# Jumpat/SegAnyGAussians

Hardware: AMD Instinct MI355X
Metric: train views/sec (fwd+bwd), 1080p, 1M Gaussians, 32-D features (higher is better)
Workload: dtype f32; 1 GPU; BASELINE cfg3: 1000000 Gaussians, 1920x1080, 32-D features, fwd+bwd, 1 view/GPU/step; parallelism=view-sharded x1

## Files before the change

### seganygaussians_amd/csrc/bin_full.h

```cpp
#pragma once

#include "blend_rec.h"
#include "common.h"
#include "cull.h"
#include "wave.h"

namespace mirast {

constexpr int BIN_MAX_WG = 256;
constexpr int BIN_THREADS = 1024;
constexpr int BIN_MAX_TILES = 22 * 1024 - 64;

__device__ __forceinline__ uint32_t slice_row(uint32_t b, uint32_t nwg)
{
    return (nwg & 7u) ? b : (b & 7u) * (nwg >> 3) + (b >> 3);
}

struct RectWork {
    uint32_t* prefix;
    uint32_t* rx;
    uint32_t* ry;
    uint32_t* wsum;
};

// ... 74 lines not shown
                getRect(rec.xy.x, rec.xy.y, (int)rec.pm, rmin, rmax, gx, gy);
                rmin.y = max(rmin.y, by0);
                rmax.y = min(rmax.y, by1);
                count = rmax.y > rmin.y ? (rmax.x - rmin.x) * (rmax.y - rmin.y) : 0u;
                s_xy[tid] = rec.xy;
                s_co[tid] = rec.co;
                s_rad[tid] = rec.pm;
                s_key[tid] = key;
            }
        }
        for_each_tile_balanced(rw, tid, rmin, rmax, count, [&](uint32_t owner, uint32_t tx, uint32_t ty) {
            const uint32_t qmask = NOCULL ? 15u : span_tile_mask(s_xy[owner], s_co[owner], (int)s_rad[owner], tx, ty, gx, gy);
            const uint32_t id = (uint32_t)(((it * 16 + (int)(owner >> 6)) * nwg + (int)blockIdx.x) * 64 + (int)(owner & 63u));
            const uint32_t slot = atomicAdd(&s_cnt[(ty - by0) * gx + tx], 1u);
            entries[slot] = make_uint2(s_key[owner], id | (qmask << ID_BITS));
        });
    }
}

__global__ void __launch_bounds__(BIN_THREADS) bin_count_kernel(int P, const BlendRec* __restrict__ index_rec,
                                                                const uint32_t* __restrict__ depth_key,
                                                                uint32_t* __restrict__ partial, uint32_t gx, uint32_t gy_all,
                                                                uint32_t by0, uint32_t by1, const int* __restrict__ r_slots,
                                                                int* __restrict__ host_r)
{
    extern __shared__ int s_grid[];
    const int tid = threadIdx.x, lane = tid & 63, wave = tid >> 6;
    if (host_r != nullptr && blockIdx.x == 0 && tid < R_SLOTS) host_r[tid * R_SLOT_STRIDE] = r_slots[tid * R_SLOT_STRIDE];
    const int stride = count_grid_stride(gx);
    const uint32_t gy = by1 - by0;
    const int cells = (int)(gy + 1) * stride;
    for (int c = tid; c < cells; c += BIN_THREADS) s_grid[c] = 0;
    __syncthreads();
    const int nwg = (int)gridDim.x;
    const int rounds = ((P + 63) / 64 + 16 * nwg - 1) / (16 * nwg);
    for (int it = 0; it < rounds; it++) {
        const int r = ((it * 16 + wave) * nwg + (int)blockIdx.x) * 64 + lane;
        if (r >= P) continue;
        if (depth_key[r] == 0xFFFFFFFFu) continue;
        const BlendRec rec = index_rec[r];
        uint2 rmin, rmax;
        getRect(rec.xy.x, rec.xy.y, (int)rec.pm, rmin, rmax, gx, gy_all);
        rmin.y = max(rmin.y, by0);
        rmax.y = min(rmax.y, by1);
        if (rmax.x <= rmin.x || rmax.y <= rmin.y) continue;
        rmin.y -= by0;
        rmax.y -= by0;
        atomicAdd(&s_grid[rmin.y * stride + rmin.x], 1);
        atomicAdd(&s_grid[rmin.y * stride + rmax.x], -1);
        atomicAdd(&s_grid[rmax.y * stride + rmin.x], -1);
        atomicAdd(&s_grid[rmax.y * stride + rmax.x], 1);
// ... 57 lines not shown
```

### seganygaussians_amd/csrc/bin_lean.h

```cpp
#pragma once

#include "blend_rec.h"
#include "common.h"
#include "cull.h"
#include "wave.h"

namespace mirast {

constexpr int BIN_LEAN_WG = 256;

__host__ __device__ inline bool band_geometry(uint32_t gx, uint32_t gy, uint32_t max_head_words, uint32_t& band_h, uint32_t& nbands)
{
    band_h = (gy + 15u) / 16u;
    if (band_h < 1u) band_h = 1u;
    while (band_h > 1u && (band_h + 1u) * (gx + 2u) > max_head_words) band_h--;
    nbands = (gy + band_h - 1u) / band_h;
    return nbands <= (uint32_t)MAX_BANDS && (band_h + 1u) * (gx + 2u) <= max_head_words;
}

__device__ __forceinline__ void band_plan(const int* __restrict__ r_slots, uint32_t nbands, uint32_t nwg, uint32_t* s_plan, int lane)
{
    uint32_t cnt = 0;
    if ((uint32_t)lane < nbands)
        for (int k = 0; k < R_SLOTS; k++) cnt += (uint32_t)r_slots[k * R_SLOT_STRIDE + R_SLOT_BANDS + lane];
    const uint32_t total = wave_sum(cnt);
    const uint32_t avail = nwg > nbands ? nwg - nbands : 0u;
    uint32_t n = (uint32_t)lane < nbands ? 1u + (total ? (uint32_t)(((uint64_t)cnt * avail) / total) : 0u) : 0u;
    if (nwg < nbands) n = (uint32_t)lane < nwg ? 1u : 0u;
    const uint32_t incl = wave_inclusive_scan(n, lane);
    if ((uint32_t)lane < nbands) s_plan[lane] = incl - n;
    if ((uint32_t)lane == nbands) s_plan[nbands] = incl;
}

constexpr int BW_WORDS = 64 * 18;
__host__ __device__ constexpr size_t span_lds_bytes(size_t head_words) { return (((head_words + 3) & ~(size_t)3) + 4 + 16 * BW_WORDS) * sizeof(uint32_t); }
constexpr uint32_t SPAN_MAX_HEAD_WORDS = 40 * 1024 - 16 * BW_WORDS - 64;

template <bool EMIT>
__global__ void __launch_bounds__(1024) bin_spans_kernel(int P, const BlendRec* __restrict__ index_rec,
                                                         const uint32_t* __restrict__ depth_key, const unsigned long long* __restrict__ band_bits,
                                                         uint32_t* __restrict__ partial, uint32_t* __restrict__ tile_total, const uint2* __restrict__ ranges,
                                                         uint2* __restrict__ entries, uint32_t gx, uint32_t gy_all,
                                                         uint32_t band_h, uint32_t nbands, const int* __restrict__ r_slots,
                                                         int* __restrict__ host_r)
{
    extern __shared__ uint32_t s_dyn[];
    __shared__ uint32_t s_plan[MAX_BANDS + 1];
    const int tid = threadIdx.x, lane = tid & 63, wave = tid >> 6;
    if (!EMIT && host_r != nullptr && blockIdx.x == 0 && tid < R_SLOTS) host_r[tid * R_SLOT_STRIDE] = r_slots[tid * R_SLOT_STRIDE];
    if (wave == 0) band_plan(r_slots, nbands, gridDim.x, s_plan, lane);
    __syncthreads();
    if (blockIdx.x >= s_plan[nbands]) return;
    uint32_t band = 0;
    while (band + 1u < nbands && s_plan[band + 1u] <= blockIdx.x) band++;
    const uint32_t nsub = s_plan[band + 1u] - s_plan[band], sub = blockIdx.x - s_plan[band];
    const uint32_t by0 = band * band_h, by1 = min(gy_all, by0 + band_h);
    const uint32_t band_bit = 1u << band;
    const uint32_t gy = by1 - by0;
    const int stride = count_grid_stride(gx);
    const int ntiles = (int)(gx * gy);
    const int tile0 = (int)(gx * by0);
    const int head = EMIT ? ((ntiles + 3) & ~3) : (((int)gy * stride + 3) & ~3);
    uint32_t* s_cnt = s_dyn;
    int* s_grid = reinterpret_cast<int*>(s_dyn);
    uint32_t* s_next = s_dyn + head;
    uint32_t* wb = s_dyn + head + 4 + wave * BW_WORDS;
    uint32_t* w_pre = wb;
    uint32_t* w_rect = wb + 64;
    uint32_t* w_key = wb + 128;
    uint32_t* w_own = wb + 192;
    float4* w_c0 = reinterpret_cast<float4*>(wb + 256);
    float4* w_c1 = reinterpret_cast<float4*>(wb + 512);
// ... 183 lines not shown
```

### seganygaussians_amd/csrc/common.h

```cpp
#pragma once

#include <hip/hip_runtime.h>
#include <stdint.h>

namespace mirast {

constexpr int R_SLOTS = 64;
constexpr int R_SLOT_STRIDE = 32;
constexpr int R_SLOT_BANDS = 4;
constexpr int MAX_BANDS = 24;
__host__ __device__ inline int count_grid_stride(uint32_t gx) { return (int)((gx + 1) | 1u); }


constexpr int TILE_X = 16;
constexpr int TILE_Y = 16;
constexpr int TILE_PIXELS = TILE_X * TILE_Y;
constexpr int BATCH = 256;
constexpr int WAVE = 64;

struct Mat3 {
    float m[3][3];
};

__device__ __forceinline__ Mat3 m3mul(const Mat3& A, const Mat3& B)
{
    Mat3 R;
#pragma unroll
    for (int c = 0; c < 3; c++)
#pragma unroll
        for (int r = 0; r < 3; r++)
            R.m[c][r] = A.m[0][r] * B.m[c][0] + A.m[1][r] * B.m[c][1] + A.m[2][r] * B.m[c][2];
    return R;
// ... 91 lines not shown
```

### seganygaussians_amd/csrc/geometry.h

```cpp
#pragma once

#include "blend_rec.h"
#include "common.h"
#include "wave.h"

namespace mirast {

__device__ constexpr float SH_C0 = 0.28209479177387814f;
__device__ constexpr float SH_C1 = 0.4886025119029199f;
__device__ constexpr float SH_C2[5] = {1.0925484305920792f, -1.0925484305920792f, 0.31539156525252005f,
                                       -1.0925484305920792f, 0.5462742152960396f};
__device__ constexpr float SH_C3[7] = {-0.5900435899266435f, 2.890611442640554f, -0.4570457994644658f,
                                       0.3731763325901154f, -0.4570457994644658f, 1.445305721320277f,
                                       -0.5900435899266435f};

__device__ __forceinline__ void computeCov3D(const float3 scale, float mod, const float4 rot, float* cov3D)
{
    Mat3 S = {{{1.0f, 0, 0}, {0, 1.0f, 0}, {0, 0, 1.0f}}};
    S.m[0][0] = mod * scale.x;
    S.m[1][1] = mod * scale.y;
    S.m[2][2] = mod * scale.z;
    float r = rot.x, x = rot.y, y = rot.z, z = rot.w;
    Mat3 R = {{{1.f - 2.f * (y * y + z * z), 2.f * (x * y - r * z), 2.f * (x * z + r * y)},
               {2.f * (x * y + r * z), 1.f - 2.f * (x * x + z * z), 2.f * (y * z - r * x)},
// ... 343 lines not shown
    for (int k = 0; k < 3; k++) {
        dL_dMt.m[0][k] *= s.x;
        dL_dMt.m[1][k] *= s.y;
        dL_dMt.m[2][k] *= s.z;
    }
    dL_drot.x = 2 * z * (dL_dMt.m[0][1] - dL_dMt.m[1][0]) + 2 * y * (dL_dMt.m[2][0] - dL_dMt.m[0][2]) + 2 * x * (dL_dMt.m[1][2] - dL_dMt.m[2][1]);
    dL_drot.y = 2 * y * (dL_dMt.m[1][0] + dL_dMt.m[0][1]) + 2 * z * (dL_dMt.m[2][0] + dL_dMt.m[0][2]) + 2 * r * (dL_dMt.m[1][2] - dL_dMt.m[2][1]) - 4 * x * (dL_dMt.m[2][2] + dL_dMt.m[1][1]);
    dL_drot.z = 2 * x * (dL_dMt.m[1][0] + dL_dMt.m[0][1]) + 2 * r * (dL_dMt.m[2][0] - dL_dMt.m[0][2]) + 2 * z * (dL_dMt.m[1][2] + dL_dMt.m[2][1]) - 4 * y * (dL_dMt.m[2][2] + dL_dMt.m[0][0]);
    dL_drot.w = 2 * r * (dL_dMt.m[0][1] - dL_dMt.m[1][0]) + 2 * x * (dL_dMt.m[2][0] + dL_dMt.m[0][2]) + 2 * y * (dL_dMt.m[1][2] + dL_dMt.m[2][1]) - 4 * z * (dL_dMt.m[1][1] + dL_dMt.m[0][0]);
}

__global__ void __launch_bounds__(256) geometry_bwd_kernel(
    int P, int D, int M, const float* __restrict__ means, const int* __restrict__ radii, const float* __restrict__ shs,
    const uint8_t* __restrict__ clamped, const float* __restrict__ scales, const float* __restrict__ rotations,
    const float* __restrict__ cov3Ds, ViewParams vp, const float* __restrict__ gpack ,
    float* __restrict__ dL_dmean2D, float* __restrict__ dL_dconics, float* __restrict__ dL_dopacity,
    float* __restrict__ dL_dmask, float* __restrict__ dL_dmeans, const float* __restrict__ dL_dcolor,
    float* __restrict__ dL_dcov, float* __restrict__ dL_dsh, float* __restrict__ dL_dscale, float* __restrict__ dL_drot)
{
    const int idx = blockIdx.x * blockDim.x + threadIdx.x;
    if (idx >= P) return;
    if (!(radii[idx] > 0)) {
        dL_dmean2D[3 * idx + 0] = dL_dmean2D[3 * idx + 1] = dL_dmean2D[3 * idx + 2] = 0.f;
        reinterpret_cast<float4*>(dL_dconics)[idx] = make_float4(0.f, 0.f, 0.f, 0.f);
        dL_dopacity[idx] = 0.f;
        if (dL_dmask) dL_dmask[idx] = 0.f;
#pragma unroll
        for (int i = 0; i < 6; i++) dL_dcov[(size_t)idx * 6 + i] = 0.f;
        dL_dmeans[3 * idx + 0] = dL_dmeans[3 * idx + 1] = dL_dmeans[3 * idx + 2] = 0.f;
        dL_dscale[3 * idx + 0] = dL_dscale[3 * idx + 1] = dL_dscale[3 * idx + 2] = 0.f;
        reinterpret_cast<float4*>(dL_drot)[idx] = make_float4(0.f, 0.f, 0.f, 0.f);
        return;
    }

    const float4 g0 = reinterpret_cast<const float4*>(gpack)[2 * idx];
    const float4 g1 = reinterpret_cast<const float4*>(gpack)[2 * idx + 1];
    dL_dmean2D[3 * idx + 0] = g0.x;
    dL_dmean2D[3 * idx + 1] = g0.y;
    dL_dmean2D[3 * idx + 2] = 0.f;
    reinterpret_cast<float4*>(dL_dconics)[idx] = make_float4(g0.z, g0.w, 0.f, g1.x);
    dL_dopacity[idx] = g1.y;
    if (dL_dmask) dL_dmask[idx] = g1.z;

    const float3 mean = make_float3(means[3 * idx], means[3 * idx + 1], means[3 * idx + 2]);
    const float3 dL_dconic = make_float3(g0.z, g0.w, g1.x);
    float cov3D[6];
#pragma unroll
    for (int i = 0; i < 6; i++) cov3D[i] = cov3Ds[(size_t)idx * 6 + i];
    Cov2DCtx c;
    cov2d_common(mean, vp, cov3D, c);
    const float h_x = vp.focal_x, h_y = vp.focal_y;
    const float limx = 1.3f * vp.tan_fovx;
    const float limy = 1.3f * vp.tan_fovy;
    const float x_grad_mul = c.txtz < -limx || c.txtz > limx ? 0 : 1;
    const float y_grad_mul = c.tytz < -limy || c.tytz > limy ? 0 : 1;
    const Mat3& T = c.T;
    const Mat3& Vrk = c.Vrk;
    const Mat3& Wm = c.W;
    const float3 t = c.t;
    const float a = c.cov.m[0][0];
    const float b = c.cov.m[0][1];
    const float cc = c.cov.m[1][1];
    const float denom = a * cc - b * b;
    float dL_da = 0, dL_db = 0, dL_dc = 0;
    const float denom2inv = 1.0f / ((denom * denom) + 0.0000001f);
    float dcov[6];
    if (denom2inv != 0) {
        dL_da = denom2inv * (-cc * cc * dL_dconic.x + 2 * b * cc * dL_dconic.y + (denom - a * cc) * dL_dconic.z);
        dL_dc = denom2inv * (-a * a * dL_dconic.z + 2 * a * b * dL_dconic.y + (denom - a * cc) * dL_dconic.x);
        dL_db = denom2inv * 2 * (b * cc * dL_dconic.x - (denom + 2 * b * b) * dL_dconic.y + a * b * dL_dconic.z);
        dcov[0] = (T.m[0][0] * T.m[0][0] * dL_da + T.m[0][0] * T.m[1][0] * dL_db + T.m[1][0] * T.m[1][0] * dL_dc);
        dcov[3] = (T.m[0][1] * T.m[0][1] * dL_da + T.m[0][1] * T.m[1][1] * dL_db + T.m[1][1] * T.m[1][1] * dL_dc);
        dcov[5] = (T.m[0][2] * T.m[0][2] * dL_da + T.m[0][2] * T.m[1][2] * dL_db + T.m[1][2] * T.m[1][2] * dL_dc);
        dcov[1] = 2 * T.m[0][0] * T.m[0][1] * dL_da + (T.m[0][0] * T.m[1][1] + T.m[0][1] * T.m[1][0]) * dL_db + 2 * T.m[1][0] * T.m[1][1] * dL_dc;
        dcov[2] = 2 * T.m[0][0] * T.m[0][2] * dL_da + (T.m[0][0] * T.m[1][2] + T.m[0][2] * T.m[1][0]) * dL_db + 2 * T.m[1][0] * T.m[1][2] * dL_dc;
        dcov[4] = 2 * T.m[0][2] * T.m[0][1] * dL_da + (T.m[0][1] * T.m[1][2] + T.m[0][2] * T.m[1][1]) * dL_db + 2 * T.m[1][1] * T.m[1][2] * dL_dc;
    } else {
#pragma unroll
        for (int i = 0; i < 6; i++) dcov[i] = 0;
    }
#pragma unroll
    for (int i = 0; i < 6; i++) dL_dcov[(size_t)idx * 6 + i] = dcov[i];

    const float dL_dT00 = 2 * (T.m[0][0] * Vrk.m[0][0] + T.m[0][1] * Vrk.m[0][1] + T.m[0][2] * Vrk.m[0][2]) * dL_da +
                          (T.m[1][0] * Vrk.m[0][0] + T.m[1][1] * Vrk.m[0][1] + T.m[1][2] * Vrk.m[0][2]) * dL_db;
    const float dL_dT01 = 2 * (T.m[0][0] * Vrk.m[1][0] + T.m[0][1] * Vrk.m[1][1] + T.m[0][2] * Vrk.m[1][2]) * dL_da +
                          (T.m[1][0] * Vrk.m[1][0] + T.m[1][1] * Vrk.m[1][1] + T.m[1][2] * Vrk.m[1][2]) * dL_db;
    const float dL_dT02 = 2 * (T.m[0][0] * Vrk.m[2][0] + T.m[0][1] * Vrk.m[2][1] + T.m[0][2] * Vrk.m[2][2]) * dL_da +
                          (T.m[1][0] * Vrk.m[2][0] + T.m[1][1] * Vrk.m[2][1] + T.m[1][2] * Vrk.m[2][2]) * dL_db;
    const float dL_dT10 = 2 * (T.m[1][0] * Vrk.m[0][0] + T.m[1][1] * Vrk.m[0][1] + T.m[1][2] * Vrk.m[0][2]) * dL_dc +
                          (T.m[0][0] * Vrk.m[0][0] + T.m[0][1] * Vrk.m[0][1] + T.m[0][2] * Vrk.m[0][2]) * dL_db;
    const float dL_dT11 = 2 * (T.m[1][0] * Vrk.m[1][0] + T.m[1][1] * Vrk.m[1][1] + T.m[1][2] * Vrk.m[1][2]) * dL_dc +
                          (T.m[0][0] * Vrk.m[1][0] + T.m[0][1] * Vrk.m[1][1] + T.m[0][2] * Vrk.m[1][2]) * dL_db;
    const float dL_dT12 = 2 * (T.m[1][0] * Vrk.m[2][0] + T.m[1][1] * Vrk.m[2][1] + T.m[1][2] * Vrk.m[2][2]) * dL_dc +
                          (T.m[0][0] * Vrk.m[2][0] + T.m[0][1] * Vrk.m[2][1] + T.m[0][2] * Vrk.m[2][2]) * dL_db;
    const float dL_dJ00 = Wm.m[0][0] * dL_dT00 + Wm.m[0][1] * dL_dT01 + Wm.m[0][2] * dL_dT02;
    const float dL_dJ02 = Wm.m[2][0] * dL_dT00 + Wm.m[2][1] * dL_dT01 + Wm.m[2][2] * dL_dT02;
    const float dL_dJ11 = Wm.m[1][0] * dL_dT10 + Wm.m[1][1] * dL_dT11 + Wm.m[1][2] * dL_dT12;
    const float dL_dJ12 = Wm.m[2][0] * dL_dT10 + Wm.m[2][1] * dL_dT11 + Wm.m[2][2] * dL_dT12;
    const float tz = 1.f / t.z;
    const float tz2 = tz * tz;
    const float tz3 = tz2 * tz;
    const float dL_dtx = x_grad_mul * -h_x * tz2 * dL_dJ02;
    const float dL_dty = y_grad_mul * -h_y * tz2 * dL_dJ12;
    const float dL_dtz = -h_x * tz2 * dL_dJ00 - h_y * tz2 * dL_dJ11 + (2 * h_x * t.x) * tz3 * dL_dJ02 + (2 * h_y * t.y) * tz3 * dL_dJ12;
// ... 43 lines not shown
```

### seganygaussians_amd/csrc/mi_rast.hip

```cpp
#include "host.h"

#include <algorithm>
#include <atomic>
#include <cstdio>
#include <cstdlib>
#include <cstring>
#include <mutex>
#include <type_traits>
#include <utility>
#include <vector>

#include "bin_full.h"
#include "bin_lean.h"
#include "tile_ranges.h"
#include "tile_sort.h"
#include "blend_bwd.h"
#include "blend_bwd_wave.h"
#include "blend_bwd_feat.h"
#include "blend_fwd.h"
#include "blend_fwd_wave.h"
#ifdef MI_RAST_PROFILING
#include "blend_fwd_x3.h"
#endif
#include "common.h"
#include "fingerprint.h"
#include "geometry.h"
// ... 1 lines not shown
#include "xcd_runs.h"
#include "xcd_stamp.h"

using namespace mirast;

namespace {

#define STAGE_CHECK(c, name)                                                                           \
    do {                                                                                               \
        hipError_t _e = hipGetLastError();                                                             \
        if (_e == hipSuccess && (c).debug) _e = hipStreamSynchronize((c).stream);                      \
        if (_e != hipSuccess)                                                                          \
            return fail(MI_RAST_ERR_HIP, std::string("[HIP ERROR] in stage ") + name + ": " + hipGetErrorString(_e)); \
    } while (0)

constexpr int MAX_DEVICES = 64;
struct HostSync {
    int* pinned = nullptr;
    int* pinned_dev = nullptr;
    uint64_t* fp = nullptr;
    uint64_t* fp_dev = nullptr;
    hipEvent_t ev = nullptr;
    hipEvent_t ev2 = nullptr;
    bool ok = false;
    const int* words() const { return pinned + R_SLOTS * R_SLOT_STRIDE; }
    int* words_dev() const { return pinned_dev + R_SLOTS * R_SLOT_STRIDE; }
    bool init()
    {
        if (ok) return true;
        if (hipHostMalloc((void**)&pinned, (R_SLOTS * R_SLOT_STRIDE + 16) * sizeof(int), hipHostMallocMapped) != hipSuccess) return false;
        if (hipHostGetDevicePointer((void**)&pinned_dev, pinned, 0) != hipSuccess) return false;
        if (hipHostMalloc((void**)&fp, (size_t)MI_FP_MAX * FP_BLOCKS * sizeof(uint64_t), hipHostMallocMapped) != hipSuccess) return false;
        if (hipHostGetDevicePointer((void**)&fp_dev, fp, 0) != hipSuccess) return false;
        if (hipEventCreateWithFlags(&ev, hipEventDisableTiming) != hipSuccess) return false;
        if (hipEventCreateWithFlags(&ev2, hipEventDisableTiming) != hipSuccess) return false;
        ok = true;
        return true;
    }
    ~HostSync()
    {
        if (ev) (void)hipEventDestroy(ev);
        if (ev2) (void)hipEventDestroy(ev2);
        if (pinned) (void)hipHostFree(pinned);
        if (fp) (void)hipHostFree(fp);
    }
};
thread_local HostSync g_host_sync_tl[MAX_DEVICES];
thread_local int g_last_longest_run[MAX_DEVICES];

int current_device()
{
    int dev = 0;
    if (hipGetDevice(&dev) != hipSuccess || dev < 0 || dev >= MAX_DEVICES) return -1;
    return dev;
// ... 289 lines not shown
    const int max_lds = (int)((BIN_MAX_TILES + 11 * 1024 + 16) * sizeof(uint32_t));
    HIP_TRY(hipFuncSetAttribute((const void*)bin_ranks_kernel<false>, hipFuncAttributeMaxDynamicSharedMemorySize, max_lds));
    HIP_TRY(hipFuncSetAttribute((const void*)bin_ranks_kernel<true>, hipFuncAttributeMaxDynamicSharedMemorySize, max_lds));
    HIP_TRY(hipFuncSetAttribute((const void*)bin_count_kernel, hipFuncAttributeMaxDynamicSharedMemorySize, max_lds));
    HIP_TRY(hipFuncSetAttribute((const void*)bin_spans_kernel<false>, hipFuncAttributeMaxDynamicSharedMemorySize, 160 * 1024 - 256));
    HIP_TRY(hipFuncSetAttribute((const void*)bin_spans_kernel<true>, hipFuncAttributeMaxDynamicSharedMemorySize, 160 * 1024 - 256));
    HIP_TRY(hipFuncSetAttribute((const void*)tile_ranges_kernel, hipFuncAttributeMaxDynamicSharedMemorySize,
                                (BIN_MAX_TILES_TOTAL + 1) * (int)sizeof(uint32_t)));
    g_attr_set[dev].store(true, std::memory_order_release);
    return MI_RAST_OK;
}

int count_and_scan_stage(const Call& c, const BinPlan& bp, const HostSync& hs)
{
    const int P = c.P, ntiles = (int)c.ntiles();
    {
        StageTimer t(c.stream, MI_STAGE_TILE_SCAN);
        if (bp.full) {
            const size_t cnt_lds = (size_t)(bp.band_rows + 1) * count_grid_stride(c.vp.grid_x) * sizeof(int);
            for (uint32_t b = 0; b < bp.nbands; b++) {
                const uint32_t by0 = b * bp.band_rows, by1 = std::min(c.vp.grid_y, by0 + bp.band_rows);
                hipLaunchKernelGGL(bin_count_kernel, dim3(bp.nwg), dim3(BIN_THREADS), cnt_lds, c.stream, P, c.geom.index_rec, c.geom.depth_key,
                                   c.img.tile_count, c.vp.grid_x, c.vp.grid_y, by0, by1, (const int*)c.img.num_rendered,
                                   b == 0 ? hs.pinned_dev : (int*)nullptr);
            }
        } else {
            hipLaunchKernelGGL(bin_spans_kernel<false>, dim3(bp.nwg), dim3(1024),
                               span_lds_bytes((size_t)bp.lean_band_h * count_grid_stride(c.vp.grid_x)), c.stream, P, c.geom.index_rec,
                               c.geom.depth_key, c.geom.band_bits, c.img.tile_count, c.img.tile_cursor, (const uint2*)nullptr, (uint2*)nullptr,
                               c.vp.grid_x, c.vp.grid_y, bp.lean_band_h, bp.lean_nbands, (const int*)c.img.num_rendered, hs.pinned_dev);
        }
        HIP_TRY(hipEventRecord(hs.ev, c.stream));
        if (bp.full)
            hipLaunchKernelGGL(scan_partials_kernel, dim3((ntiles + 63) / 64), dim3(1024), 0, c.stream, ntiles, bp.nwg,
                               c.img.tile_count, c.img.tile_cursor);
        const uint32_t run_cap = !(c.flags & MI_RAST_EQUAL_RUNS) ? (uint32_t)RUN_MODEL_CAP : 0u;
        hipLaunchKernelGGL(tile_ranges_kernel, dim3(1), dim3(1024),
                           ((size_t)std::min(ntiles, BIN_MAX_TILES_TOTAL) + 1) * sizeof(uint32_t), c.stream, ntiles, c.img.tile_cursor,
                           c.img.ranges, c.img.words(), (const int*)c.img.num_rendered, hs.words_dev(), c.img.tile_consumed, c.img.tile_nsurv,
                           c.img.run_bounds, run_cap, (uint32_t)RUN_MODEL_FIX);
    }
    STAGE_CHECK(c, "tile scan");
    return MI_RAST_OK;
}

int emit_stage(const Call& c, const BinPlan& bp, int R)
{
    const int P = c.P, ntiles = (int)c.ntiles();
    const bool verify = !bp.full && (c.flags & MI_RAST_VERIFY_LISTS) != 0;
    if (verify) HIP_TRY(hipMemsetAsync(c.bin.entries, 0, (size_t)R * sizeof(uint2), c.stream));
    {
        StageTimer t(c.stream, MI_STAGE_EMIT);
        if (bp.full) {
            const size_t band_tiles = (size_t)bp.band_rows * c.vp.grid_x;
            const size_t emit_lds = ((size_t)((band_tiles + 3) & ~(size_t)3) + 11 * 1024 + 16) * sizeof(uint32_t);
            for (uint32_t b = 0; b < bp.nbands; b++) {
                const uint32_t by0 = b * bp.band_rows, by1 = std::min(c.vp.grid_y, by0 + bp.band_rows);
                with_bool(bp.nocull, [&](auto nocull) {
                    hipLaunchKernelGGL(bin_ranks_kernel<decltype(nocull)::value>, dim3(bp.nwg), dim3(BIN_THREADS), emit_lds, c.stream, P, c.geom.index_rec,
                                       c.geom.depth_key, c.img.tile_count, c.img.ranges, c.bin.entries, c.vp.grid_x, c.vp.grid_y, by0, by1);
                });
            }
        } else {
            hipLaunchKernelGGL(bin_spans_kernel<true>, dim3(bp.nwg), dim3(1024), span_lds_bytes((size_t)bp.lean_band_h * c.vp.grid_x), c.stream,
                               P, c.geom.index_rec, c.geom.depth_key, c.geom.band_bits, c.img.tile_count, c.img.tile_cursor, c.img.ranges, c.bin.entries,
                               c.vp.grid_x, c.vp.grid_y, bp.lean_band_h, bp.lean_nbands, (const int*)c.img.num_rendered, (int*)nullptr);
        }
    }
    STAGE_CHECK(c, "emit entries");
    if (verify) {
        uint32_t* ctr = reinterpret_cast<uint32_t*>(c.img.words() + NR_VERIFY);
        HIP_TRY(hipMemsetAsync(ctr, 0, sizeof(uint32_t), c.stream));
        hipLaunchKernelGGL(verify_entries_kernel, dim3(ntiles), dim3(256), 0, c.stream, (uint32_t)ntiles, c.img.ranges, c.bin.entries, ctr);
        uint32_t unwritten = 0;
        HIP_TRY(hipMemcpyAsync(&unwritten, ctr, sizeof(uint32_t), hipMemcpyDeviceToHost, c.stream));
        HIP_TRY(hipStreamSynchronize(c.stream));
        if (unwritten)
            return fail(MI_RAST_ERR_HIP, "internal error: " + std::to_string(unwritten) + " list slots were counted but not emitted "
                                         "(count / emit passes of bin_spans_kernel disagree)");
    }
    return MI_RAST_OK;
}

int take_longest_run(Call& c, const HostSync& hs, int dev)
{
    HIP_TRY(hipEventSynchronize(hs.ev2));
    c.longest_run = longest_of(hs.words() + NR_RUN_BOUNDS, c.ntiles());
    g_last_longest_run[dev] = (int)c.longest_run;
    return MI_RAST_OK;
}

template <int CLASS>
void launch_tile_sort_wave(const Call& c)
{
    hipLaunchKernelGGL(tile_sort_wave_kernel<CLASS>, dim3((c.ntiles() + 3) / 4), dim3(256), 0, c.stream, c.ntiles(), c.img.ranges,
                       (const uint2*)c.bin.entries, c.bin.blend_list);
}
template <int LO, int CAP, bool FB, int NT>
void launch_tile_sort(const Call& c)
{
    hipLaunchKernelGGL((tile_sort_kernel<LO, CAP, FB, NT>), dim3(c.ntiles()), dim3(NT), 0, c.stream, c.ntiles(), c.img.ranges, c.bin.entries,
                       c.bin.scratch, (const int*)(c.img.words() + NR_KEY_BITS), c.bin.blend_list);
// ... 12 lines not shown
        if (max_tile_count > 2048) launch_tile_sort_wave<2>(c);
        if (max_tile_count > TILE_SORT_WAVE_MAX) launch_tile_sort<TILE_SORT_WAVE_MAX, 6144, false, 1024>(c);
        if (max_tile_count > 6144) launch_tile_sort<6144, 8192, true, 1024>(c);
    }
    STAGE_CHECK(c, "tile sort");
    return MI_RAST_OK;
}

int geometry_and_binning(Call& c, const FrontArgs& a, int* num_rendered)
{
    const int dev = current_device();
    if (dev < 0) return fail(MI_RAST_ERR_HIP, "hipGetDevice failed (or device ordinal >= 64)");
    HostSync& hs = g_host_sync_tl[dev];
    BinPlan bp;
    if (int rc = plan_binning(c, bp)) return rc;
    size_t goff[MI_GEOM_NFIELDS], ioff[MI_IMG_NFIELDS], boff[MI_BIN_NFIELDS];
    char* geom_base = a.geometry_buffer(mi_rast_geometry_layout(c.P, goff), a.geometry_user);
    if (!geom_base) return fail(MI_RAST_ERR_ALLOC, "geometry buffer callback returned NULL");
    c.geom = geom_from(geom_base, c.P);
    char* img_base = a.image_buffer(mi_rast_image_layout(c.vp.W, c.vp.H, ioff), a.image_user);
    if (!img_base) return fail(MI_RAST_ERR_ALLOC, "image buffer callback returned NULL");
    c.img = img_from(img_base, c.vp.W, c.vp.H);

    if (int rc = preprocess_stage(c, a, bp)) return rc;
    if (int rc = opt_in_to_large_lds(dev)) return rc;
    if (!hs.init()) return fail(MI_RAST_ERR_HIP, "cannot allocate pinned host buffer / event");
    if (int rc = count_and_scan_stage(c, bp, hs)) return rc;
    HIP_TRY(hipEventRecord(hs.ev2, c.stream));
    HIP_TRY(hipEventSynchronize(hs.ev));
    long long Rsum = 0;
    for (int k = 0; k < R_SLOTS; k++) Rsum += hs.pinned[k * R_SLOT_STRIDE];
    if (Rsum > 0x7fffffffll) return fail(MI_RAST_ERR_INVALID, "more than 2^31 tile overlaps");
    const int R = (int)Rsum;
    *num_rendered = R;

    char* bin_base = a.binning_buffer(mi_rast_binning_layout(R, boff), a.binning_user);
    if (!bin_base) return fail(MI_RAST_ERR_ALLOC, "binning buffer callback returned NULL");
    c.bin = bin_from(bin_base, R);
    if (R == 0) return take_longest_run(c, hs, dev);
    if (int rc = emit_stage(c, bp, R)) return rc;
    return sort_stage(c, bp, hs, dev, R);
}

struct FwdArgs { int channels; const float *features, *mask, *bg; float *out_color, *out_mask, *out_depth; };
struct BwdArgs { int channels; const float *bg, *colors, *dL_dpix, *dL_dout_mask; float* dL_dcolor; };

template <int C, int EXTRA>
void launch_blend_fwd(const Call& c, const FwdArgs& a, ChannelBlock b)
{
    constexpr bool MAY_BE_PARTIAL = C == 16 && EXTRA == 0;
    with_bools(MAY_BE_PARTIAL && b.real < C, c.xexp(), [&](auto partial, auto xexp) {
        if constexpr (MAY_BE_PARTIAL || !decltype(partial)::value)
            hipLaunchKernelGGL((blend_fwd_kernel<C, EXTRA, decltype(xexp)::value, decltype(partial)::value>), dim3(c.vp.grid_x, c.vp.grid_y), dim3(256), 0,
                               c.stream, c.img.ranges, c.bin.blend_list, c.geom.index_rec, c.vp.W, c.vp.H, a.features + b.c0, a.mask, c.geom.depths,
// ... 522 lines not shown
```

### seganygaussians_amd/rasterizer.py

```python
from __future__ import annotations

import contextlib
import math
import os
import ctypes as C
import threading
from typing import NamedTuple

import torch
import torch.nn as nn

from . import _lib
from ._ffi import check, contig, dev_ptr, stream_ptr
from .geometry_cache import GeometryCache, disable_geometry_cache, enable_geometry_cache, geometry_cache


def cpu_deep_copy_tuple(input_tuple):
    copied_tensors = [item.cpu().clone() if isinstance(item, torch.Tensor) else item for item in input_tuple]
    return tuple(copied_tensors)


class GaussianRasterizationSettings(NamedTuple):
    image_height: int
    image_width: int
# ... 181 lines not shown
    if background is None or background.numel() < channels:
        raise RuntimeError(f"bg must hold one value per channel: {0 if background is None else background.numel()} given, "
                           f"{channels} channels rendered")
    if colors is not None and colors.numel() != 0 and P != 0 and (colors.ndimension() != 2 or colors.size(0) != P
                                                                  or colors.size(1) != channels):
        raise RuntimeError(f"colors_precomp must have dimensions (num_points, {channels}); got {tuple(colors.shape)}")


def set_features_ready_event(event) -> None:
    _opts.features_ready = event


def _flags_of(geomBuffer, flags):
    if flags is not None:
        return flags
    notes = getattr(geomBuffer, "mi_notes", None)
    return 0 if notes is None else notes.flags


def rasterize_gaussians_backward_native(channels, with_mask_depth, background, means3D, radii, colors, scales,
                                        rotations, scale_modifier, cov3D_precomp, viewmatrix, projmatrix, tan_fovx,
                                        tan_fovy, dL_dout_color, dL_dout_mask, sh, degree, campos, geomBuffer, R,
                                        binningBuffer, imageBuffer, debug, flags=None, prezeroed=None, pack_zeroed=None,
                                        features_only=False):
    L = _lib.load()
    P = means3D.size(0)
    H, W = dL_dout_color.size(1), dL_dout_color.size(2)
    M = sh.size(1) if sh.numel() != 0 else 0
    dev = means3D.device
    _check_widths(channels, background, colors, P)
    if dL_dout_color.ndimension() != 3 or dL_dout_color.size(0) != channels:
        raise RuntimeError(f"dL_dout_color must have dimensions ({channels}, H, W); got {tuple(dL_dout_color.shape)}")
    if features_only and (with_mask_depth or colors.numel() == 0):
        raise RuntimeError("features_only backward needs precomputed colours and the plain (not DEPTH) rasterizer")
    full = not features_only
    o = dict(device=dev, dtype=torch.float32)
    g = {}
    if full:
        shapes = [("dL_dmeans3D", (P, 3)), ("dL_dmeans2D", (P, 3)), ("dL_dconic", (P, 2, 2)), ("dL_dopacity", (P, 1)),
                  ("dL_dcov3D", (P, 6)), ("dL_dscales", (P, 3)), ("dL_drotations", (P, 4))]
        if with_mask_depth:
            shapes.append(("dL_dmask", (P, 1)))
        counts = [math.prod(shp) for _, shp in shapes]
        starts = [0]
        for n in counts:
            starts.append(starts[-1] + (n + 3) // 4 * 4)
        flat = torch.empty(starts[-1], **o)
        if debug:
            flat.fill_(float("nan"))
        for (name, shp), n, off in zip(shapes, counts, starts):
            g[name] = flat[off:off + n].view(shp)
    if pack_zeroed is None:
        pack_zeroed = prezeroed is not None
    if prezeroed is not None and (tuple(prezeroed.shape) != (P, channels) or prezeroed.device != dev or (debug and full)):
        prezeroed = None
    g["dL_dcolors"] = prezeroed if prezeroed is not None else torch.zeros((P, channels), **o)
    if full:
        g["dL_dsh"] = torch.zeros((P, M, 3), **o)
    if P != 0:
        def only_full(x):
            return x if full else None

        def grad(name, present=True):
            return g[name].data_ptr() if (present and name in g) else None

        t = [contig(x) for x in (background, means3D, only_full(sh), colors, only_full(scales), only_full(rotations),
                                  only_full(cov3D_precomp), viewmatrix, projmatrix, campos, dL_dout_color,
                                  dL_dout_mask if with_mask_depth else None, radii)]
        bg_c, m3_c, sh_c, col_c, sc_c, rot_c, cov_c, vm_c, pm_c, cp_c, dpix_c, dmask_c, radii_c = t
        with torch.cuda.device(dev):
            rc = L.mi_rast_backward(
                P, int(degree), int(M) if full else 0, int(channels), int(R), dev_ptr(bg_c, "bg", dev), W, H,
                dev_ptr(m3_c, "means3D", dev), dev_ptr(sh_c, "sh", dev), dev_ptr(col_c, "colors_precomp", dev),
                dev_ptr(sc_c, "scales", dev), float(scale_modifier), dev_ptr(rot_c, "rotations", dev),
                dev_ptr(cov_c, "cov3D_precomp", dev), dev_ptr(vm_c, "viewmatrix", dev),
                dev_ptr(pm_c, "projmatrix", dev), dev_ptr(cp_c, "campos", dev), float(tan_fovx), float(tan_fovy),
                dev_ptr(radii_c, "radii", dev, torch.int32), geomBuffer.data_ptr(), binningBuffer.data_ptr(),
                imageBuffer.data_ptr(), dev_ptr(dpix_c, "dL_dout_color", dev), dev_ptr(dmask_c, "dL_dout_mask", dev),
                grad("dL_dmeans2D"), grad("dL_dconic"), grad("dL_dopacity"), grad("dL_dcolors"), grad("dL_dmask"),
                grad("dL_dmeans3D"), grad("dL_dcov3D"), grad("dL_dsh", M > 0), grad("dL_dscales"), grad("dL_drotations"),
                int(bool(debug)) if full else 0,
                int(_flags_of(geomBuffer, flags)) | (0 if full else _lib.MI_RAST_BWD_FEATURES_ONLY)
                | (_lib.MI_RAST_PREZERO_BWD if pack_zeroed else 0), stream_ptr(dev))
        check(rc)
    if features_only:
        return None, g["dL_dcolors"], None, None, None, None, None, None
    if with_mask_depth:
        return (g["dL_dmeans2D"], g["dL_dcolors"], g["dL_dopacity"], g["dL_dmask"], g["dL_dmeans3D"], g["dL_dcov3D"], g["dL_dsh"],
                g["dL_dscales"], g["dL_drotations"])
    return (g["dL_dmeans2D"], g["dL_dcolors"], g["dL_dopacity"], g["dL_dmeans3D"], g["dL_dcov3D"], g["dL_dsh"], g["dL_dscales"],
            g["dL_drotations"])


def mark_visible_native(means3D, viewmatrix, projmatrix):
    L = _lib.load()
    P = means3D.size(0)
    dev = means3D.device
    present = torch.zeros(P, dtype=torch.bool, device=dev)
    if P != 0:
        m3_c, vm_c, pm_c = contig(means3D), contig(viewmatrix), contig(projmatrix)
        with torch.cuda.device(dev):
            rc = L.mi_rast_mark_visible(P, dev_ptr(m3_c, "means3D", dev), dev_ptr(vm_c, "viewmatrix", dev),
                                        dev_ptr(pm_c, "projmatrix", dev), present.data_ptr(), stream_ptr(dev))
        check(rc)
    return present


def rasterize_mask_gaussians_native(means3D, opacity, mask, scales, rotations, scale_modifier, cov3D_precomp,
                                    viewmatrix, projmatrix, tan_fovx, tan_fovy, image_height, image_width,
                                    prefiltered, debug):
    _opts.features_ready = None
    if means3D.ndimension() != 2 or means3D.size(1) != 3:
        raise RuntimeError("means3D must have dimensions (num_points, 3)")
# ... 109 lines not shown
                                  binningBuffer, imgBuffer)
            ctx.mark_non_differentiable(radii)
            ctx.set_materialize_grads(False)
            ctx.out_shape = tuple(color.shape)
            return color, radii

        @staticmethod
        def backward(ctx, grad_out_color, _):
            num_rendered = ctx.num_rendered
            rs = ctx.raster_settings
            if grad_out_color is None:
                grad_out_color = torch.zeros(ctx.out_shape, dtype=torch.float32, device=ctx.saved_tensors[1].device)
            (colors_precomp, means3D, scales, rotations, cov3Ds_precomp, radii, sh, geomBuffer, binningBuffer,
             imgBuffer) = ctx.saved_tensors
            args = (rs.bg, means3D, radii, colors_precomp, scales, rotations, rs.scale_modifier, cov3Ds_precomp,
                    rs.viewmatrix, rs.projmatrix, rs.tanfovx, rs.tanfovy, grad_out_color, sh, rs.sh_degree, rs.campos,
                    geomBuffer, num_rendered, binningBuffer, imgBuffer, rs.debug)
            prezeroed, pack_zeroed = ctx.mi_notes.claim()
            feat_only = _features_only_applies(channels, colors_precomp, ctx.needs_input_grad, rs.debug)
            (grad_means2D, grad_colors_precomp, grad_opacities, grad_means3D, grad_cov3Ds_precomp, grad_sh,
             grad_scales, grad_rotations) = _snapshot_call(
                rs.debug, args, lambda *a: rasterize_gaussians_backward_native(
                    channels, False, *a[:13], None, *a[13:], flags=ctx.mi_notes.flags, prezeroed=prezeroed,
                    pack_zeroed=pack_zeroed, features_only=feat_only), *_SNAPSHOT_BW)
            return (grad_means3D, grad_means2D, grad_sh, grad_colors_precomp, grad_opacities, grad_scales,
                    grad_rotations, grad_cov3Ds_precomp, None)

    def rasterize_gaussians(means3D, means2D, sh, colors_precomp, opacities, scales, rotations, cov3Ds_precomp,
                            raster_settings):
        _opts.grad_mode = torch.is_grad_enabled()
        try:
            return _RasterizeGaussians.apply(means3D, means2D, sh, colors_precomp, opacities, scales, rotations,
                                             cov3Ds_precomp, raster_settings)
        finally:
            _opts.grad_mode = True

    class GaussianRasterizer(_RasterizerModule):
        def forward(self, means3D, means2D, opacities, shs=None, colors_precomp=None, scales=None, rotations=None,
                    cov3D_precomp=None):
            _one_of_colors(shs, colors_precomp)
            _one_of_cov(scales, rotations, cov3D_precomp)
            shs, colors_precomp, scales, rotations, cov3D_precomp = _or_empty(shs, colors_precomp, scales, rotations, cov3D_precomp)
            return rasterize_gaussians(means3D, means2D, shs, colors_precomp, opacities, scales, rotations,
                                       cov3D_precomp, self.raster_settings)

    return _RasterizeGaussians, rasterize_gaussians, GaussianRasterizer

# ... 18 lines not shown
            ctx.save_for_backward(colors_precomp, means3D, scales, rotations, cov3Ds_precomp, radii, sh, geomBuffer,
                                  binningBuffer, imgBuffer)
            ctx.mark_non_differentiable(radii)
            ctx.set_materialize_grads(False)
            ctx.out_shapes = (tuple(color.shape), tuple(out_mask.shape))
            return color, out_mask, depth, radii

        @staticmethod
        def backward(ctx, grad_out_color, grad_out_mask, grad_out_depth, _):
            num_rendered = ctx.num_rendered
            rs = ctx.raster_settings
            dev_ = ctx.saved_tensors[1].device
            if grad_out_color is None:
                grad_out_color = torch.zeros(ctx.out_shapes[0], dtype=torch.float32, device=dev_)
            if grad_out_mask is None:
                grad_out_mask = torch.zeros(ctx.out_shapes[1], dtype=torch.float32, device=dev_)
            (colors_precomp, means3D, scales, rotations, cov3Ds_precomp, radii, sh, geomBuffer, binningBuffer,
             imgBuffer) = ctx.saved_tensors
            args = (rs.bg, means3D, radii, colors_precomp, scales, rotations, rs.scale_modifier, cov3Ds_precomp,
                    rs.viewmatrix, rs.projmatrix, rs.tanfovx, rs.tanfovy, grad_out_color, grad_out_mask, sh,
                    rs.sh_degree, rs.campos, geomBuffer, num_rendered, binningBuffer, imgBuffer, rs.debug)
            (grad_means2D, grad_colors_precomp, grad_opacities, grad_mask, grad_means3D, grad_cov3Ds_precomp, grad_sh,
             grad_scales, grad_rotations) = _snapshot_call(
                rs.debug, args, lambda *a: rasterize_gaussians_backward_native(channels, True, *a, flags=ctx.mi_notes.flags),
                *_SNAPSHOT_BW)
            grad_mask = grad_mask.view(ctx.mask_shape)
            return (grad_means3D, grad_means2D, grad_sh, grad_colors_precomp, grad_opacities, grad_mask, grad_scales,
                    grad_rotations, grad_cov3Ds_precomp, None)

    class _RasterizeMaskGaussians(torch.autograd.Function):
        @staticmethod
        def forward(ctx, means3D, means2D, opacities, mask, scales, rotations, cov3Ds_precomp, raster_settings):
            rs = raster_settings
            num_rendered, out_mask, radii, geomBuffer, binningBuffer, imgBuffer = rasterize_mask_gaussians_native(
                means3D, opacities, mask, scales, rotations, rs.scale_modifier, cov3Ds_precomp, rs.viewmatrix,
                rs.projmatrix, rs.tanfovx, rs.tanfovy, rs.image_height, rs.image_width, rs.prefiltered, rs.debug)
            ctx.raster_settings = rs
            ctx.num_rendered = num_rendered
            ctx.mask_shape = mask.shape
            ctx.mi_notes = _take_notes(geomBuffer)
            ctx.save_for_backward(means3D, means2D, opacities, scales, rotations, cov3Ds_precomp, radii, geomBuffer,
                                  binningBuffer, imgBuffer)
            ctx.mark_non_differentiable(radii)
            ctx.set_materialize_grads(False)
            ctx.out_shape = tuple(out_mask.shape)
            return out_mask, radii

# ... 86 lines not shown
```

Before: 915.8 views/s.

## Poll generation-tagged pinned slots for num_rendered and skip unused conic/cov3D gradients

The count kernels now publish each per-slot rendered count to mapped host memory as a 64-bit word tagged with a generation number. The host spins briefly on those words instead of waiting on an event recorded after the count pass, falling back to the later event if the values do not arrive within the spin window. This is meant to shorten the forward-pass stall before the host learns the list size. Separately, the backward pass no longer allocates or writes the dL_dconic buffer, and skips dL_dcov3D when no precomputed covariances are supplied, which cuts memory traffic and allocation. The spin adds host CPU busy-waiting and relies on system-scope relaxed stores becoming visible in order.

```diff
diff --git a/seganygaussians_amd/csrc/bin_full.h b/seganygaussians_amd/csrc/bin_full.h
--- a/seganygaussians_amd/csrc/bin_full.h
+++ b/seganygaussians_amd/csrc/bin_full.h
@@ -120,11 +120,11 @@
                                                                 const uint32_t* __restrict__ depth_key,
                                                                 uint32_t* __restrict__ partial, uint32_t gx, uint32_t gy_all,
                                                                 uint32_t by0, uint32_t by1, const int* __restrict__ r_slots,
-                                                                int* __restrict__ host_r)
+                                                                int* __restrict__ host_r, uint32_t host_gen)
 {
     extern __shared__ int s_grid[];
     const int tid = threadIdx.x, lane = tid & 63, wave = tid >> 6;
-    if (host_r != nullptr && blockIdx.x == 0 && tid < R_SLOTS) host_r[tid * R_SLOT_STRIDE] = r_slots[tid * R_SLOT_STRIDE];
+    if (host_r != nullptr && blockIdx.x == 0 && tid < R_SLOTS) publish_r_slot(host_r, tid, r_slots[tid * R_SLOT_STRIDE], host_gen);
     const int stride = count_grid_stride(gx);
     const uint32_t gy = by1 - by0;
     const int cells = (int)(gy + 1) * stride;
diff --git a/seganygaussians_amd/csrc/bin_lean.h b/seganygaussians_amd/csrc/bin_lean.h
--- a/seganygaussians_amd/csrc/bin_lean.h
+++ b/seganygaussians_amd/csrc/bin_lean.h
@@ -42,12 +42,12 @@
                                                          uint32_t* __restrict__ partial, uint32_t* __restrict__ tile_total, const uint2* __restrict__ ranges,
                                                          uint2* __restrict__ entries, uint32_t gx, uint32_t gy_all,
                                                          uint32_t band_h, uint32_t nbands, const int* __restrict__ r_slots,
-                                                         int* __restrict__ host_r)
+                                                         int* __restrict__ host_r, uint32_t host_gen)
 {
     extern __shared__ uint32_t s_dyn[];
     __shared__ uint32_t s_plan[MAX_BANDS + 1];
     const int tid = threadIdx.x, lane = tid & 63, wave = tid >> 6;
-    if (!EMIT && host_r != nullptr && blockIdx.x == 0 && tid < R_SLOTS) host_r[tid * R_SLOT_STRIDE] = r_slots[tid * R_SLOT_STRIDE];
+    if (!EMIT && host_r != nullptr && blockIdx.x == 0 && tid < R_SLOTS) publish_r_slot(host_r, tid, r_slots[tid * R_SLOT_STRIDE], host_gen);
     if (wave == 0) band_plan(r_slots, nbands, gridDim.x, s_plan, lane);
     __syncthreads();
     if (blockIdx.x >= s_plan[nbands]) return;
diff --git a/seganygaussians_amd/csrc/common.h b/seganygaussians_amd/csrc/common.h
--- a/seganygaussians_amd/csrc/common.h
+++ b/seganygaussians_amd/csrc/common.h
@@ -8,6 +8,11 @@
 constexpr int R_SLOTS = 64;
 constexpr int R_SLOT_STRIDE = 32;
 constexpr int R_SLOT_BANDS = 4;
+__device__ __forceinline__ void publish_r_slot(int* host_r, int k, int partial_sum, uint32_t generation)
+{
+    const unsigned long long w = (unsigned long long)(uint32_t)partial_sum | ((unsigned long long)generation << 32);
+    __hip_atomic_store(reinterpret_cast<unsigned long long*>(host_r + k * R_SLOT_STRIDE), w, __ATOMIC_RELAXED, __HIP_MEMORY_SCOPE_SYSTEM);
+}
 constexpr int MAX_BANDS = 24;
 __host__ __device__ inline int count_grid_stride(uint32_t gx) { return (int)((gx + 1) | 1u); }
 
diff --git a/seganygaussians_amd/csrc/geometry.h b/seganygaussians_amd/csrc/geometry.h
--- a/seganygaussians_amd/csrc/geometry.h
+++ b/seganygaussians_amd/csrc/geometry.h
@@ -389,11 +389,13 @@
     if (idx >= P) return;
     if (!(radii[idx] > 0)) {
         dL_dmean2D[3 * idx + 0] = dL_dmean2D[3 * idx + 1] = dL_dmean2D[3 * idx + 2] = 0.f;
-        reinterpret_cast<float4*>(dL_dconics)[idx] = make_float4(0.f, 0.f, 0.f, 0.f);
+        if (dL_dconics) reinterpret_cast<float4*>(dL_dconics)[idx] = make_float4(0.f, 0.f, 0.f, 0.f);
         dL_dopacity[idx] = 0.f;
         if (dL_dmask) dL_dmask[idx] = 0.f;
-#pragma unroll
-        for (int i = 0; i < 6; i++) dL_dcov[(size_t)idx * 6 + i] = 0.f;
+        if (dL_dcov) {
+#pragma unroll
+            for (int i = 0; i < 6; i++) dL_dcov[(size_t)idx * 6 + i] = 0.f;
+        }
         dL_dmeans[3 * idx + 0] = dL_dmeans[3 * idx + 1] = dL_dmeans[3 * idx + 2] = 0.f;
         dL_dscale[3 * idx + 0] = dL_dscale[3 * idx + 1] = dL_dscale[3 * idx + 2] = 0.f;
         reinterpret_cast<float4*>(dL_drot)[idx] = make_float4(0.f, 0.f, 0.f, 0.f);
@@ -405,7 +407,7 @@
     dL_dmean2D[3 * idx + 0] = g0.x;
     dL_dmean2D[3 * idx + 1] = g0.y;
     dL_dmean2D[3 * idx + 2] = 0.f;
-    reinterpret_cast<float4*>(dL_dconics)[idx] = make_float4(g0.z, g0.w, 0.f, g1.x);
+    if (dL_dconics) reinterpret_cast<float4*>(dL_dconics)[idx] = make_float4(g0.z, g0.w, 0.f, g1.x);
     dL_dopacity[idx] = g1.y;
     if (dL_dmask) dL_dmask[idx] = g1.z;
 
@@ -446,8 +448,10 @@
 #pragma unroll
         for (int i = 0; i < 6; i++) dcov[i] = 0;
     }
-#pragma unroll
-    for (int i = 0; i < 6; i++) dL_dcov[(size_t)idx * 6 + i] = dcov[i];
+    if (dL_dcov) {
+#pragma unroll
+        for (int i = 0; i < 6; i++) dL_dcov[(size_t)idx * 6 + i] = dcov[i];
+    }
 
     const float dL_dT00 = 2 * (T.m[0][0] * Vrk.m[0][0] + T.m[0][1] * Vrk.m[0][1] + T.m[0][2] * Vrk.m[0][2]) * dL_da +
                           (T.m[1][0] * Vrk.m[0][0] + T.m[1][1] * Vrk.m[0][1] + T.m[1][2] * Vrk.m[0][2]) * dL_db;
diff --git a/seganygaussians_amd/csrc/mi_rast.hip b/seganygaussians_amd/csrc/mi_rast.hip
--- a/seganygaussians_amd/csrc/mi_rast.hip
+++ b/seganygaussians_amd/csrc/mi_rast.hip
@@ -2,6 +2,7 @@
 
 #include <algorithm>
 #include <atomic>
+#include <chrono>
 #include <cstdio>
 #include <cstdlib>
 #include <cstring>
@@ -49,7 +50,9 @@
     uint64_t* fp_dev = nullptr;
     hipEvent_t ev = nullptr;
     hipEvent_t ev2 = nullptr;
+    uint32_t generation = 0;
     bool ok = false;
+    uint32_t next_generation() { return ++generation ? generation : ++generation; }
     const int* words() const { return pinned + R_SLOTS * R_SLOT_STRIDE; }
     int* words_dev() const { return pinned_dev + R_SLOTS * R_SLOT_STRIDE; }
     bool init()
@@ -57,6 +60,7 @@
         if (ok) return true;
         if (hipHostMalloc((void**)&pinned, (R_SLOTS * R_SLOT_STRIDE + 16) * sizeof(int), hipHostMallocMapped) != hipSuccess) return false;
         if (hipHostGetDevicePointer((void**)&pinned_dev, pinned, 0) != hipSuccess) return false;
+        memset(pinned, 0, (R_SLOTS * R_SLOT_STRIDE + 16) * sizeof(int));
         if (hipHostMalloc((void**)&fp, (size_t)MI_FP_MAX * FP_BLOCKS * sizeof(uint64_t), hipHostMallocMapped) != hipSuccess) return false;
         if (hipHostGetDevicePointer((void**)&fp_dev, fp, 0) != hipSuccess) return false;
         if (hipEventCreateWithFlags(&ev, hipEventDisableTiming) != hipSuccess) return false;
@@ -392,15 +396,15 @@
                 const uint32_t by0 = b * bp.band_rows, by1 = std::min(c.vp.grid_y, by0 + bp.band_rows);
                 hipLaunchKernelGGL(bin_count_kernel, dim3(bp.nwg), dim3(BIN_THREADS), cnt_lds, c.stream, P, c.geom.index_rec, c.geom.depth_key,
                                    c.img.tile_count, c.vp.grid_x, c.vp.grid_y, by0, by1, (const int*)c.img.num_rendered,
-                                   b == 0 ? hs.pinned_dev : (int*)nullptr);
+                                   b == 0 ? hs.pinned_dev : (int*)nullptr, hs.generation);
             }
         } else {
             hipLaunchKernelGGL(bin_spans_kernel<false>, dim3(bp.nwg), dim3(1024),
                                span_lds_bytes((size_t)bp.lean_band_h * count_grid_stride(c.vp.grid_x)), c.stream, P, c.geom.index_rec,
                                c.geom.depth_key, c.geom.band_bits, c.img.tile_count, c.img.tile_cursor, (const uint2*)nullptr, (uint2*)nullptr,
-                               c.vp.grid_x, c.vp.grid_y, bp.lean_band_h, bp.lean_nbands, (const int*)c.img.num_rendered, hs.pinned_dev);
+                               c.vp.grid_x, c.vp.grid_y, bp.lean_band_h, bp.lean_nbands, (const int*)c.img.num_rendered, hs.pinned_dev,
+                               hs.generation);
         }
-        HIP_TRY(hipEventRecord(hs.ev, c.stream));
         if (bp.full)
             hipLaunchKernelGGL(scan_partials_kernel, dim3((ntiles + 63) / 64), dim3(1024), 0, c.stream, ntiles, bp.nwg,
                                c.img.tile_count, c.img.tile_cursor);
@@ -434,7 +438,7 @@
         } else {
             hipLaunchKernelGGL(bin_spans_kernel<true>, dim3(bp.nwg), dim3(1024), span_lds_bytes((size_t)bp.lean_band_h * c.vp.grid_x), c.stream,
                                P, c.geom.index_rec, c.geom.depth_key, c.geom.band_bits, c.img.tile_count, c.img.tile_cursor, c.img.ranges, c.bin.entries,
-                               c.vp.grid_x, c.vp.grid_y, bp.lean_band_h, bp.lean_nbands, (const int*)c.img.num_rendered, (int*)nullptr);
+                               c.vp.grid_x, c.vp.grid_y, bp.lean_band_h, bp.lean_nbands, (const int*)c.img.num_rendered, (int*)nullptr, 0u);
         }
     }
     STAGE_CHECK(c, "emit entries");
@@ -448,6 +452,40 @@
         if (unwritten)
             return fail(MI_RAST_ERR_HIP, "internal error: " + std::to_string(unwritten) + " list slots were counted but not emitted "
                                          "(count / emit passes of bin_spans_kernel disagree)");
+    }
+    return MI_RAST_OK;
+}
+
+constexpr int READBACK_SPIN_US = 200;
+int read_back_R(const HostSync& hs, long long& Rsum)
+{
+    HIP_TRY(hipEventSynchronize(hs.ev));
+    const auto slot = [&](int k) {
+        return __atomic_load_n(reinterpret_cast<const unsigned long long*>(hs.pinned + k * R_SLOT_STRIDE), __ATOMIC_ACQUIRE);
+    };
+    const auto deadline = std::chrono::steady_clock::now() + std::chrono::microseconds(READBACK_SPIN_US);
+    Rsum = 0;
+    for (int k = 0; k < R_SLOTS;) {
+        const unsigned long long w = slot(k);
+        if ((uint32_t)(w >> 32) == hs.generation) {
+            Rsum += (int)(uint32_t)w;
+            k++;
+            continue;
+        }
+        if (std::chrono::steady_clock::now() < deadline) {
+#if defined(__x86_64__) || defined(__i386__)
+            __builtin_ia32_pause();
+#endif
+            continue;
+        }
+        HIP_TRY(hipEventSynchronize(hs.ev2));
+        Rsum = 0;
+        for (int j = 0; j < R_SLOTS; j++) {
+            const unsigned long long v = slot(j);
+            if ((uint32_t)(v >> 32) != hs.generation) return fail(MI_RAST_ERR_HIP, "internal error: the count pass did not hand over num_rendered");
+            Rsum += (int)(uint32_t)v;
+        }
+        break;
     }
     return MI_RAST_OK;
 }
@@ -506,14 +544,15 @@
     if (!img_base) return fail(MI_RAST_ERR_ALLOC, "image buffer callback returned NULL");
     c.img = img_from(img_base, c.vp.W, c.vp.H);
 
+    if (!hs.init()) return fail(MI_RAST_ERR_HIP, "cannot allocate pinned host buffer / event");
+    if (int rc = opt_in_to_large_lds(dev)) return rc;
     if (int rc = preprocess_stage(c, a, bp)) return rc;
-    if (int rc = opt_in_to_large_lds(dev)) return rc;
-    if (!hs.init()) return fail(MI_RAST_ERR_HIP, "cannot allocate pinned host buffer / event");
+    HIP_TRY(hipEventRecord(hs.ev, c.stream));
+    hs.next_generation();
     if (int rc = count_and_scan_stage(c, bp, hs)) return rc;
     HIP_TRY(hipEventRecord(hs.ev2, c.stream));
-    HIP_TRY(hipEventSynchronize(hs.ev));
     long long Rsum = 0;
-    for (int k = 0; k < R_SLOTS; k++) Rsum += hs.pinned[k * R_SLOT_STRIDE];
+    if (int rc = read_back_R(hs, Rsum)) return rc;
     if (Rsum > 0x7fffffffll) return fail(MI_RAST_ERR_INVALID, "more than 2^31 tile overlaps");
     const int R = (int)Rsum;
     *num_rendered = R;
diff --git a/seganygaussians_amd/rasterizer.py b/seganygaussians_amd/rasterizer.py
--- a/seganygaussians_amd/rasterizer.py
+++ b/seganygaussians_amd/rasterizer.py
@@ -227,7 +227,7 @@
                                         rotations, scale_modifier, cov3D_precomp, viewmatrix, projmatrix, tan_fovx,
                                         tan_fovy, dL_dout_color, dL_dout_mask, sh, degree, campos, geomBuffer, R,
                                         binningBuffer, imageBuffer, debug, flags=None, prezeroed=None, pack_zeroed=None,
-                                        features_only=False):
+                                        features_only=False, want_cov3D=True):
     L = _lib.load()
     P = means3D.size(0)
     H, W = dL_dout_color.size(1), dL_dout_color.size(2)
@@ -242,8 +242,9 @@
     o = dict(device=dev, dtype=torch.float32)
     g = {}
     if full:
-        shapes = [("dL_dmeans3D", (P, 3)), ("dL_dmeans2D", (P, 3)), ("dL_dconic", (P, 2, 2)), ("dL_dopacity", (P, 1)),
-                  ("dL_dcov3D", (P, 6)), ("dL_dscales", (P, 3)), ("dL_drotations", (P, 4))]
+        want_cov3D = bool(want_cov3D) or cov3D_precomp.numel() != 0
+        shapes = [("dL_dmeans3D", (P, 3)), ("dL_dmeans2D", (P, 3)), ("dL_dopacity", (P, 1))] + \
+                 ([("dL_dcov3D", (P, 6))] if want_cov3D else []) + [("dL_dscales", (P, 3)), ("dL_drotations", (P, 4))]
         if with_mask_depth:
             shapes.append(("dL_dmask", (P, 1)))
         counts = [math.prod(shp) for _, shp in shapes]
@@ -282,7 +283,7 @@
                 dev_ptr(pm_c, "projmatrix", dev), dev_ptr(cp_c, "campos", dev), float(tan_fovx), float(tan_fovy),
                 dev_ptr(radii_c, "radii", dev, torch.int32), geomBuffer.data_ptr(), binningBuffer.data_ptr(),
                 imageBuffer.data_ptr(), dev_ptr(dpix_c, "dL_dout_color", dev), dev_ptr(dmask_c, "dL_dout_mask", dev),
-                grad("dL_dmeans2D"), grad("dL_dconic"), grad("dL_dopacity"), grad("dL_dcolors"), grad("dL_dmask"),
+                grad("dL_dmeans2D"), None, grad("dL_dopacity"), grad("dL_dcolors"), grad("dL_dmask"),
                 grad("dL_dmeans3D"), grad("dL_dcov3D"), grad("dL_dsh", M > 0), grad("dL_dscales"), grad("dL_drotations"),
                 int(bool(debug)) if full else 0,
                 int(_flags_of(geomBuffer, flags)) | (0 if full else _lib.MI_RAST_BWD_FEATURES_ONLY)
@@ -291,9 +292,9 @@
     if features_only:
         return None, g["dL_dcolors"], None, None, None, None, None, None
     if with_mask_depth:
-        return (g["dL_dmeans2D"], g["dL_dcolors"], g["dL_dopacity"], g["dL_dmask"], g["dL_dmeans3D"], g["dL_dcov3D"], g["dL_dsh"],
+        return (g["dL_dmeans2D"], g["dL_dcolors"], g["dL_dopacity"], g["dL_dmask"], g["dL_dmeans3D"], g.get("dL_dcov3D"), g["dL_dsh"],
                 g["dL_dscales"], g["dL_drotations"])
-    return (g["dL_dmeans2D"], g["dL_dcolors"], g["dL_dopacity"], g["dL_dmeans3D"], g["dL_dcov3D"], g["dL_dsh"], g["dL_dscales"],
+    return (g["dL_dmeans2D"], g["dL_dcolors"], g["dL_dopacity"], g["dL_dmeans3D"], g.get("dL_dcov3D"), g["dL_dsh"], g["dL_dscales"],
             g["dL_drotations"])
 
 
@@ -449,7 +450,7 @@
              grad_scales, grad_rotations) = _snapshot_call(
                 rs.debug, args, lambda *a: rasterize_gaussians_backward_native(
                     channels, False, *a[:13], None, *a[13:], flags=ctx.mi_notes.flags, prezeroed=prezeroed,
-                    pack_zeroed=pack_zeroed, features_only=feat_only), *_SNAPSHOT_BW)
+                    pack_zeroed=pack_zeroed, features_only=feat_only, want_cov3D=cov3Ds_precomp.numel() != 0), *_SNAPSHOT_BW)
             return (grad_means3D, grad_means2D, grad_sh, grad_colors_precomp, grad_opacities, grad_scales,
                     grad_rotations, grad_cov3Ds_precomp, None)
 
@@ -514,7 +515,8 @@
                     rs.sh_degree, rs.campos, geomBuffer, num_rendered, binningBuffer, imgBuffer, rs.debug)
             (grad_means2D, grad_colors_precomp, grad_opacities, grad_mask, grad_means3D, grad_cov3Ds_precomp, grad_sh,
              grad_scales, grad_rotations) = _snapshot_call(
-                rs.debug, args, lambda *a: rasterize_gaussians_backward_native(channels, True, *a, flags=ctx.mi_notes.flags),
+                rs.debug, args, lambda *a: rasterize_gaussians_backward_native(channels, True, *a, flags=ctx.mi_notes.flags,
+                                                                               want_cov3D=cov3Ds_precomp.numel() != 0),
                 *_SNAPSHOT_BW)
             grad_mask = grad_mask.view(ctx.mask_shape)
             return (grad_means3D, grad_means2D, grad_sh, grad_colors_precomp, grad_opacities, grad_mask, grad_scales,
```

Result: no change. 923.0 views/s, median of 6 (+0.8%).
